# zwpku/colvars-finder

Measured on AMD Instinct MI355X. Metric: MD frames/sec through EigenFunctionTask train step, higher is better.
Workload: dtype f32; 1 GPU; BASELINE config 3: alanine-dipeptide-shaped EigenFunctionTask, generator mode, k=3, 22 atoms, align+position features d_r=66, nets [66,20,20,20,1], diag_coeff, Adam; frames_per_gpu=100000, batch_per_gpu=20000, global_batch=20000, parallelism=dp1 (frames sharded; all-reduce of batch sums + flat gradient)

## Files before the change

colvars-finder_amd/csrc/cvf_common.hpp:

```cpp
#pragma once
#include <hip/hip_runtime.h>
#include <stdint.h>
#include "cvf.h"

#define CVF_WAVE 64

void cvf_set_error(const char* fmt, ...);
int cvf_check_launch(const char* what);

#define CVF_REQUIRE(cond, ...)      \
  do {                              \
    if (!(cond)) {                  \
      cvf_set_error(__VA_ARGS__);   \
      return -1;                    \
    }                               \
  } while (0)

static inline int64_t cvf_ntiles(int64_t B) { return (B + CVF_TILE - 1) / CVF_TILE; }
static inline int cvf_cu_count() {
  static const int n = [] {
    int dev = 0, v = 0;
    if (hipGetDevice(&dev) != hipSuccess || hipDeviceGetAttribute(&v, hipDeviceAttributeMultiprocessorCount, dev) != hipSuccess || v < 1) v = 256;
    return v;
  }();
// ... 76 lines not shown

#ifdef CVF_STAMPS
#ifndef CVF_STAMP_WPB
#define CVF_STAMP_WPB 2
#endif
static __device__ unsigned long long g_stamps[64 * 4096];
#define CVF_STAMP(i)                                                                              \
  do {                                                                                            \
    if ((threadIdx.x & 63) == 0 && blockIdx.y == 0 && blockIdx.z == 0 && blockIdx.x < 4096 && (threadIdx.x >> 6) < CVF_STAMP_WPB)   \
      g_stamps[(blockIdx.x * CVF_STAMP_WPB + (threadIdx.x >> 6)) % 4096 * 64 + (i)] = __builtin_amdgcn_s_memtime(); \
  } while (0)
#define CVF_STAMP_RT(i)                                                                           \
  do {                                                                                            \
    if ((threadIdx.x & 63) == 0 && blockIdx.y == 0 && blockIdx.z == 0 && blockIdx.x < 4096 && (threadIdx.x >> 6) < CVF_STAMP_WPB)   \
      g_stamps[(blockIdx.x * CVF_STAMP_WPB + (threadIdx.x >> 6)) % 4096 * 64 + (i)] = __builtin_amdgcn_s_memrealtime(); \
  } while (0)
#else
#define CVF_STAMP(i) do {} while (0)
#define CVF_STAMP_RT(i) do {} while (0)
#endif

__host__ __device__ __forceinline__ int x_tile_stride(int nc) { return (nc & 3) == 2 ? nc : (nc | 1); }

template <int kBatch = 18>
__device__ __forceinline__ void load_x_tile(const float* __restrict__ x, int64_t B, int nc, int64_t tile, float* lds,
                                            int tid, int nthreads = CVF_WAVE, int frames = CVF_TILE) {
  const int stride = x_tile_stride(nc);
  const int64_t f0 = tile * frames;
  const int total = frames * nc;
  if (f0 + frames <= B) {
    const float4* src = reinterpret_cast<const float4*>(x + f0 * nc);
    const int nvec = total >> 2;
    int e = tid * 4;
    int fr = e / nc;
    int j = e - fr * nc;
    const int step = 4 * nthreads;
    const int dfr = step / nc, dj = step - dfr * nc;
    if (stride == nc) {
      float4* dst = reinterpret_cast<float4*>(lds);
      for (int v0 = tid; v0 < nvec; v0 += nthreads * kBatch) {
        float4 val[kBatch];
#pragma unroll
        for (int i = 0; i < kBatch; ++i) {
          const int v = v0 + nthreads * i;
          val[i] = src[v < nvec ? v : nvec - 1];
        }
#pragma unroll
// ... 9 lines not shown
#pragma unroll
      for (int i = 0; i < kBatch; ++i) {
        const int v = v0 + nthreads * i;
        val[i] = src[v < nvec ? v : nvec - 1];
      }
#pragma unroll
      for (int i = 0; i < kBatch; ++i) {
        if (v0 + nthreads * i < nvec) {
          int f = fr, jj = j;
          lds[f * stride + jj] = val[i].x;
          if (++jj == nc) { jj = 0; ++f; }
          lds[f * stride + jj] = val[i].y;
          if (++jj == nc) { jj = 0; ++f; }
          lds[f * stride + jj] = val[i].z;
          if (++jj == nc) { jj = 0; ++f; }
          lds[f * stride + jj] = val[i].w;
        }
        fr += dfr;
        j += dj;
        if (j >= nc) { j -= nc; ++fr; }
      }
    }
  } else {
    for (int e = tid; e < total; e += nthreads) {
      int fr = e / nc;
      int j = e - fr * nc;
      int64_t src = f0 + fr;
      if (src > B - 1) src = B - 1;
      lds[fr * stride + j] = x[src * nc + j];
    }
  }
}

__device__ __forceinline__ void lds_barrier() { asm volatile("s_waitcnt lgkmcnt(0)\n\ts_barrier" ::: "memory"); }

typedef float f2 __attribute__((ext_vector_type(2)));
__device__ __forceinline__ f2 splat2(float v) { return f2{v, v}; }
__device__ __forceinline__ f2 fma2(f2 a, f2 b, f2 c) { return __builtin_elementwise_fma(a, b, c); }

struct V3 {
  float x, y, z;
};
__device__ __forceinline__ V3 v3(float x, float y, float z) { return V3{x, y, z}; }
__device__ __forceinline__ V3 operator+(V3 a, V3 b) { return V3{a.x + b.x, a.y + b.y, a.z + b.z}; }
__device__ __forceinline__ V3 operator-(V3 a, V3 b) { return V3{a.x - b.x, a.y - b.y, a.z - b.z}; }
__device__ __forceinline__ V3 operator*(float s, V3 a) { return V3{s * a.x, s * a.y, s * a.z}; }
__device__ __forceinline__ float dot(V3 a, V3 b) { return a.x * b.x + a.y * b.y + a.z * b.z; }
__device__ __forceinline__ V3 cross(V3 a, V3 b) {
  return V3{a.y * b.z - a.z * b.y, a.z * b.x - a.x * b.z, a.x * b.y - a.y * b.x};
}

__device__ __forceinline__ V3 row_times(V3 v, const float* R) {
// ... 12 lines not shown
```

colvars-finder_amd/csrc/ef16_back.hip:

```cpp
#include "ef16_common.hpp"

namespace {

struct Back16Args {
  int k;
  int64_t B;
  int64_t n_tiles;
  int64_t T;
  const float* w_lag;
};
struct Back16Nets {
  int D;
  int n_params;
  int base[CVF_MAX_NETS];
};
template <int H, int NH>
__host__ __device__ constexpr int net_w_off(int l, int hd) { return l == 0 ? 0 : hd + H + (l - 1) * (H * H + H); }
template <int H, int NH>
__host__ __device__ constexpr int net_b_off(int l, int hd) { return net_w_off<H, NH>(l, hd) + (l == 0 ? hd : l == NH ? H : H * H); }

template <int H, int NH, bool MULTI, bool GEN>
__global__ __launch_bounds__(256, 4) void ef16_back_kernel(Back16Args args, Back16Nets nets, const float* __restrict__ theta,
                                                            const float* __restrict__ packed, const float* __restrict__ w,
                                                            const float* __restrict__ feat, const float* __restrict__ y_tiled,
// ... 111 lines not shown
  };

  int64_t tile = blockIdx.x;
  do {
    if constexpr (MULTI) {
      asm volatile("" : "+s"(D), "+s"(k));
      derive();
      asm volatile("" : "+v"(lane));
      derive_lane();
    }
    CVF_STAMP(8);
    double crow[CVF_MAX_NETS];
#pragma unroll
    for (int j = 0; j < CVF_MAX_NETS; ++j) crow[j] = coef[k + net * k + (j < k ? j : k - 1)];
    double gS1n = coef[net], gEtn = coef[k + k * k + net];
    double gS1ln = GEN ? 0.0 : coef[2 * k + k * k + net], gS2ln = GEN ? 0.0 : coef[3 * k + k * k + net];
    __builtin_amdgcn_sched_barrier(0);
    const bool lagged = !GEN && tile >= args.T;
    const int64_t t0 = lagged ? tile - args.T : tile;
    const int64_t frame = t0 * CVF_TILE + fo;
    const bool valid = frame < args.B;
    const float wraw = w[valid ? frame : args.B - 1];
    float yb[CVF_MAX_NETS];
#pragma unroll
    for (int j = 0; j < CVF_MAX_NETS; ++j) yb[j] = y_tiled[(t0 * k + (j < k ? j : k - 1)) * CVF_TILE + fo];
    float ylag = 0.0f, wlraw = 0.0f;
    if constexpr (!GEN) {
      ylag = y_tiled[((args.T + t0) * k + net) * CVF_TILE + fo];
      wlraw = args.w_lag[valid ? frame : args.B - 1];
    }
    const URows sv = urows(saved + (tile * k + net) * (int64_t)(kHand<NH>() * NG * 256) + wave * 64, kHand<NH>() * NG * 256 - wave * 64, lane);
    Vec<H, 1> h[NH], e[NH > 1 ? NH - 1 : 1], t[NH];
#pragma unroll
    for (int l = 0; l < NH; ++l) {
#pragma unroll
      for (int rt = 0; rt < RT; ++rt) h[l].v[rt][0] = f32x4{0.0f, 0.0f, 0.0f, 0.0f};
#pragma unroll
      for (int g = 0; g < NG; ++g) h[l].v[g >> 2][0][g & 3] = sv.ld((l * NG + g) * 256);
    }
    if constexpr (GEN) {
#pragma unroll
      for (int l = 0; l + 1 < NH; ++l) {
#pragma unroll
        for (int rt = 0; rt < RT; ++rt) e[l].v[rt][0] = f32x4{0.0f, 0.0f, 0.0f, 0.0f};
#pragma unroll
        for (int g = 0; g < NG; ++g) e[l].v[g >> 2][0][g & 3] = sv.ld(((NH + l) * NG + g) * 256);
      }
#pragma unroll
// ... 147 lines not shown
          for (int pr = wave; pr < RTO * CTH; pr += WPB) {
            const int rt = pr / CTH, ct = pr - rt * CTH;
            emit_tile(l, H, rt, ct, outer2(SA1, SB1, SA2, SB2, rt, ct));
          }
        }
        if (l == NH - 1) emit_last();
        __syncthreads();
      } else {
        if (strip) {
#pragma unroll
          for (int c = 0; c < 4; ++c) {
            if (c < ncol) {
              const float xv = c == nfeat ? 1.0f : xs[c < 3 ? c : 2];
              const float qv = c == nfeat ? 0.0f : gamma * qs[c < 3 ? c : 2];
              const float pick = strip_rows<H>([&](int rt, int r) {
                if constexpr (GEN) return fmaf(zbar.v[rt][0][r], xv, dl.v[rt][0][r] * qv);
                else return zbar.v[rt][0][r] * xv;
              }, col);
              if (col < NG && rowf < H) SB1[(wave * H + rowf) * 4 + c] = pick;
            }
          }
        }
        __syncthreads();
        auto half0 = [&](f32x4 (&acc)[RTO], const float* SA, const float4 (&b)[4], int ct, int rt0, int rstep, bool ones) {
          const int i = 16 * ct + row16;
          const float pad = (ones && i == D) ? 1.0f : 0.0f;
#pragma unroll
          for (int rt = 0; rt < RTO; ++rt) {
            if (rt >= rt0 && (rt - rt0) % rstep == 0) {
              const float4* a1 = reinterpret_cast<const float4*>(SA + (16 * rt + row16) * kPitch + 4 * q);
              float4 av[4];
#pragma unroll
              for (int j = 0; j < 4; ++j) av[j] = a1[4 * j];
#pragma unroll
              for (int j = 0; j < 4; ++j) {
                acc[rt] = mfma4(av[j].x, i < D ? b[j].x : pad, acc[rt]);
                acc[rt] = mfma4(av[j].y, i < D ? b[j].y : pad, acc[rt]);
                acc[rt] = mfma4(av[j].z, i < D ? b[j].z : pad, acc[rt]);
                acc[rt] = mfma4(av[j].w, i < D ? b[j].w : pad, acc[rt]);
              }
            }
          }
        };
        const int extra = (CTM - WPB) * RTO;
        f32x4 acc[RTO];
#pragma unroll
        for (int rt = 0; rt < RTO; ++rt) acc[rt] = f32x4{0.0f, 0.0f, 0.0f, 0.0f};
        auto tail0 = [&](f32x4& tacc, const float* SA, const float4 (&b)[4], int ct, bool ones) {
          const int i = 16 * ct + row16;
          const float pad = (ones && i == D) ? 1.0f : 0.0f;
          const float4* a1 = reinterpret_cast<const float4*>(SA + (16 + (lane & 3)) * kPitch + 4 * q);
          float4 av[4];
#pragma unroll
          for (int j = 0; j < 4; ++j) av[j] = a1[4 * j];
#pragma unroll
          for (int j = 0; j < 4; ++j) {
            tacc = mfma1(av[j].x, i < D ? b[j].x : pad, tacc);
            tacc = mfma1(av[j].y, i < D ? b[j].y : pad, tacc);
            tacc = mfma1(av[j].z, i < D ? b[j].z : pad, tacc);
            tacc = mfma1(av[j].w, i < D ? b[j].w : pad, tacc);
          }
        };
        if (wave < CTM) {
          f32x4 tacc = {0.0f, 0.0f, 0.0f, 0.0f};
          half0(acc, SA1, bA, wave, 0, TAIL4 ? RTO : 1, true);
          if constexpr (TAIL4) tail0(tacc, SA1, bA, wave, true);
          if (wave < extra) request(bA, f_tile, WPB + wave / RTO);
          if constexpr (GEN) {
            half0(acc, SA2, bB, wave, 0, TAIL4 ? RTO : 1, false);
            if constexpr (TAIL4) tail0(tacc, SA2, bB, wave, false);
          }
#pragma unroll
          for (int rt = 0; rt < (TAIL4 ? 1 : RTO); ++rt) emit_tile(0, D, rt, wave, acc[rt]);
          if constexpr (TAIL4) {
            const float v = rows_sum_scatter(tacc);
            int o = 16 + q;
            asm volatile("" : "+v"(o));
            const int i = 16 * wave + row16;
            const bool isw = o < H && i < D, isb = o < H && i == D;
            emit_entry(isw || isb, isw ? o * D + i : HD + (o < H ? o : 0), v);
          }
        }
        for (int pr = wave; pr < extra; pr += WPB) {
          const int ct = WPB + pr / RTO, rt = pr % RTO;
          if (pr != wave || wave >= CTM) request(bA, f_tile, ct);
          if constexpr (GEN) request(bB, q_tile, ct);
#pragma unroll
          for (int r_ = 0; r_ < RTO; ++r_) acc[r_] = f32x4{0.0f, 0.0f, 0.0f, 0.0f};
          half0(acc, SA1, bA, ct, rt, RTO, true);
          if constexpr (GEN) half0(acc, SA2, bB, ct, rt, RTO, false);
#pragma unroll
          for (int r_ = 0; r_ < RTO; ++r_)
            if (r_ == rt) emit_tile(0, D, r_, ct, acc[r_]);
        }
        emit_strip();
        if (NH == 1) emit_last();
        __syncthreads();
      }
    }
    tile += gridDim.x;
  } while (MULTI && tile < args.n_tiles);
  CVF_STAMP(17);
  if (MULTI) {
    __syncthreads();
    for (int i = tid; i < gspan; i += NT) out[i] = GI[i];
  }
  if (step != nullptr && blockIdx.x == 0 && blockIdx.y == 0 && tid == 0) *step += 1;
  CVF_STAMP(18);
}

}

extern "C" int64_t cvf_ef16_backward_slab_rows(int64_t n_tiles) { return n_tiles < 1024 ? n_tiles : 1024; }
// ... 74 lines not shown
```

colvars-finder_amd/csrc/ef16_front_kernel.hpp:

```cpp
#pragma once
#include "ef16_common.hpp"
#include "cvf_p2p.hpp"

namespace {
constexpr int kRowsUnit = kU * kAuxP;
static_assert(kRowsUnit % 4 == 0, "a unit's alignment rows are staged as 16-byte pieces");

template <bool kTransfer>
__device__ __forceinline__ void ef16_align_unit(const float* my, const float* refL, const int nal, const int lane, float* auxL,
                                                float* rsL) {
  const int f = lane >> 2, p = lane & 3;
  double acc[15];
#pragma unroll
  for (int i = 0; i < 15; ++i) acc[i] = 0.0;
#pragma unroll 2
  for (int b = p; b < nal; b += 4) {
    const double x0 = (double)my[3 * b], x1 = (double)my[3 * b + 1], x2 = (double)my[3 * b + 2];
    const double r0 = (double)refL[3 * b], r1 = (double)refL[3 * b + 1], r2 = (double)refL[3 * b + 2];
    acc[0] += x0; acc[1] += x1; acc[2] += x2;
    acc[3] = fma(x0, r0, acc[3]); acc[4] = fma(x0, r1, acc[4]); acc[5] = fma(x0, r2, acc[5]);
    acc[6] = fma(x1, r0, acc[6]); acc[7] = fma(x1, r1, acc[7]); acc[8] = fma(x1, r2, acc[8]);
    acc[9] = fma(x2, r0, acc[9]); acc[10] = fma(x2, r1, acc[10]); acc[11] = fma(x2, r2, acc[11]);
    acc[12] += r0; acc[13] += r1; acc[14] += r2;
  }
// ... 5 lines not shown
#pragma unroll
  for (int i = 0; i < 3; ++i)
#pragma unroll
    for (int j = 0; j < 3; ++j) Hm[i][j] = fma(-cd[i], acc[12 + j], acc[3 + 3 * i + j]);
  KabschOut ko;
  if constexpr (kTransfer) {
    kabsch_from_H<false>(Hm, ko);
#pragma unroll
    for (int i = 0; i < 6; ++i) ko.Kinv[i] = 0.0f;
  } else {
    kabsch_from_H<true>(Hm, ko);
  }
  const Centre c = centre_of(cd);
  const float av[kAuxP] = {ko.R[0], ko.R[1], ko.R[2], ko.R[3], ko.R[4], ko.R[5], ko.R[6], ko.R[7], ko.R[8], c.hi[0], c.hi[1], c.hi[2],
                           ko.Kinv[0], ko.Kinv[1], ko.Kinv[2], ko.Kinv[3], ko.Kinv[4], ko.Kinv[5], c.lo[0], c.lo[1], c.lo[2]};
#pragma unroll
  for (int i = 0; i < kAuxP; ++i)
    if ((i & 3) == p) auxL[f * kAuxP + i] = av[i];
  if (lane < 3) rsL[lane] = (float)(lane == 0 ? acc[12] : lane == 1 ? acc[13] : acc[14]);
}

__device__ __forceinline__ V3 ef16_feature(const float* my, const int at, const Centre& c, const float* R) {
  return row_times(centred(my, at, c), R);
}

template <int H, int NH, int NIT, bool ALLAL, bool ROWS = false>
__global__ __launch_bounds__(1024, 4) void ef16_front_kernel(cvf_mlp_desc mlp, const float* __restrict__ theta,
                                                             const float* __restrict__ packed, cvf_pp_desc pp,
                                                             const float* __restrict__ x, int64_t B,
                                                             const float* __restrict__ a, const float* __restrict__ w,
                                                             float* __restrict__ feat_tiled, float* __restrict__ y_tiled,
                                                             float* __restrict__ saved, float* __restrict__ q_tiled,
                                                             float* __restrict__ e_tiled, double* __restrict__ partial, int launch,
                                                             const float* __restrict__ x_lag, int64_t units_x,
                                                             const float* __restrict__ w_lag, const float* __restrict__ rows) {
  static_assert(!ROWS || NIT > 0, "alignment rows: generator instances only");
  constexpr int RT = Hid<H>::RT, NG = Hid<H>::NG, SMAX = 18, CTMAX = 5;
  constexpr bool kTransfer = NIT == 0;
  extern __shared__ __attribute__((aligned(16))) float lds_all[];
  const int upb = launch & 0xff;
  const int k = mlp.n_nets, D = mlp.dims[0];
  const int wave_b = __builtin_amdgcn_readfirstlane((int)threadIdx.x >> 6);
  const int usub = upb > 1 ? wave_b / k : 0;
  const int wave = wave_b - usub * k;
  const int tid = (int)threadIdx.x - usub * (64 * k), lane_in = tid & 63;
  const int nthreads = upb > 1 ? 64 * k : (int)blockDim.x, nw = nthreads >> 6;
// ... 74 lines not shown
    const int64_t frame = unit * kU + (tid < kU ? tid : kU - 1);
    const float wv_ld = *(w != nullptr ? w + (frame < B ? frame : B - 1) : rows);
    const float wv = (w != nullptr && frame < B) ? wv_ld : 0.0f;
    {
      const float* ft = feat_tiled + tile * (int64_t)D * CVF_TILE + kU * sub + col;
#pragma unroll
      for (int s = 0; s < SMAX; ++s) {
        const int kf = 4 * (s < S ? s : S - 1) + q;
        bf0[s] = ft[(kf < D ? kf : D - 1) * CVF_TILE];
      }
    }
    request_a0();
    float4* adst = reinterpret_cast<float4*>(auxL);
    if (tid < n4r) adst[tid] = row_a;
    if (tid + nthreads < n4r) adst[tid + nthreads] = row_b;
    if (tid < 3) rsL[tid] = rs_in;
    if (iso) {
    } else if (plain) {
      float4* dst = reinterpret_cast<float4*>(xt);
      if (tid < n4) dst[tid] = cx0;
      if (tid + nthreads < n4) dst[tid + nthreads] = cx1;
      for (int v = tid + 2 * nthreads; v < n4; v += nthreads) dst[v] = xsrc[v];
    } else {
      load_x_tile<6>(x, B, nc, unit, xt, tid, nthreads, kU);
    }
    if (tid < nt) refL[tid] = tv;
    for (int j = tid + nthreads; j < nt; j += nthreads) refL[j] = j < 3 * nal ? pp.ref_c[j] : (a != nullptr ? a[j - 3 * nal] : 0.0f);
    if (tid < kU) wL[tid] = wv;
    request_bias0();
  } else {
  if (stride == nc && (unit + 1) * kU <= B && (reinterpret_cast<uintptr_t>(x) & 15) == 0) {
    const float4* src = reinterpret_cast<const float4*>(x + unit * (int64_t)(kU * nc));
    float4* dst = reinterpret_cast<float4*>(xt);
    const int n4 = (kU * nc) >> 2;
    for (int v = tid; v < n4; v += nthreads) dst[v] = src[v];
  } else {
    load_x_tile<6>(x, B, nc, unit, xt, tid, nthreads, kU);
  }
  for (int j = tid; j < 3 * nal + nc; j += nthreads) refL[j] = j < 3 * nal ? pp.ref_c[j] : (a != nullptr ? a[j - 3 * nal] : 0.0f);
  if (tid < kU) {
    const int64_t frame = unit * kU + tid;
    wL[tid] = (w != nullptr && frame < B) ? w[frame] : 0.0f;
  }
  if (wave != 0) request_layer0();
  __syncthreads();
  }
  const float* my = xt + f * stride;
// ... 6 lines not shown
    }
    lds_barrier();
  }
  CVF_STAMP(22);

  if constexpr (!ROWS) {
    float R[9];
    const float* ar = auxL + f * kAuxP;
#pragma unroll
    for (int i = 0; i < 9; ++i) R[i] = ar[i];
    Centre c;
#pragma unroll
    for (int i = 0; i < 3; ++i) {
      c.hi[i] = ar[9 + i];
      c.lo[i] = ar[18 + i];
    }
    for (int at = p + 4 * wave; at < N; at += 4 * nw) {
      const V3 al = ef16_feature(my, at, c, R);
      float* fi = featI + f * kImgP + 3 * at;
      fi[0] = al.x;
      fi[1] = al.y;
      fi[2] = al.z;
    }
    lds_barrier();
  }
  CVF_STAMP(23);

  Vec<H, 1> h[NH];
  auto set_bias = [&](Vec<H, 1>& X, const float (&b)[RT][4]) {
#pragma unroll
    for (int rt = 0; rt < RT; ++rt)
#pragma unroll
      for (int r = 0; r < 4; ++r) X.v[rt][0][r] = b[rt][r];
  };
  set_bias(h[0], bias[0]);
  {
    float bf[SMAX];
    float* fr = featI + col * kImgP;
    static_assert(4 * (SMAX - 1) + 3 < kImgP, "the ROWS twins' feature copy stays inside a frame's row of the image");
    unsigned own = 0u;
    if constexpr (ROWS) {
      if (iso) {
        const int P = nw >= 8 ? 8 : nw >= 4 ? 4 : nw >= 2 ? 2 : 1;
        own = (P == 8 ? 0x10101u : P == 4 ? 0x11111u : P == 2 ? 0x15555u : 0x3ffffu) << (wave & (P - 1));
      }
    }
#pragma unroll
    for (int s = 0; s < SMAX; ++s) {
      const int kf = 4 * (s < S ? s : S - 1) + q;
      if constexpr (ROWS) bf[s] = bf0[s];
      else bf[s] = fr[kf < D ? kf : D - 1];
    }
    HFrag<H> hf[NH > 1 ? NH - 1 : 1];
#pragma unroll
    for (int l = 1; l < NH; ++l) {
      load_hfrag_u<H>(hf[l - 1], pk, L.fh(l));
      load_hid_const_u<H>(urows(theta + mlp.b_off[net][l], H, q), bias[l]);
    }
#pragma unroll
    for (int s = 0; s < SMAX; ++s) {
      if (s < S) {
#pragma unroll
        for (int rt = 0; rt < RT; ++rt) h[0].v[rt][0] = mfma4(a0[s][rt], bf[s], h[0].v[rt][0]);
        if constexpr (ROWS) {
          if ((own >> s) & 1u) fr[q + 4 * s] = bf[s];
        }
      }
    }
    CVF_STAMP(24);
    tanh_inplace<H, 1>(h[0]);
#pragma unroll
    for (int l = 1; l < NH; ++l) {
      set_bias(h[l], bias[l]);
      hidden_mul<H, 1>(h[l], hf[l - 1], h[l - 1]);
      tanh_inplace<H, 1>(h[l]);
    }
  }
  float wl[RT][4];
  load_hid_const_u<H>(urows(theta + mlp.w_off[net][NH], H, q), wl);
  const float bL = theta[mlp.b_off[net][NH]];
  HFrag<H> tf[NH > 1 ? NH - 1 : 1];
#pragma unroll
  for (int l = 1; l < NH; ++l) load_hfrag_u<H>(tf[l - 1], pk, L.th(l));

  const URows sv = urows(saved + (tile * k + net) * (int64_t)(kHand<NH>() * NG * 256) + sub * 64, kHand<NH>() * NG * 256 - sub * 64, lane);
  {
    float part = 0.0f;
#pragma unroll
    for (int rt = 0; rt < RT; ++rt)
#pragma unroll
      for (int r = 0; r < 4; ++r) part = fmaf(wl[rt][r], h[NH - 1].v[rt][0][r], part);
    const float yv = sum_over_q(part) + bL;
    yL[net * kU + col] = yv;
    y_tiled[(tile * k + net) * CVF_TILE + kU * sub + col] = yv;
  }
  CVF_STAMP(25);
  if constexpr (kTransfer) {
#pragma unroll
    for (int l = 0; l < NH; ++l)
#pragma unroll
      for (int g = 0; g < NG; ++g) sv.st((l * NG + g) * 256, h[l].v[g >> 2][0][g & 3]);
    float* ft = feat_tiled + tile * (int64_t)D * CVF_TILE + kU * sub + f;
    const float* fi = featI + f * kImgP;
#pragma unroll 1
    for (int j = p + 4 * wave; j < D; j += 4 * nw) ft[j * CVF_TILE] = fi[j];
    return;
  } else {

  {
    float t0[CTMAX][NG];
#pragma unroll
    for (int rt = 0; rt < CTMAX; ++rt)
#pragma unroll
      for (int s = 0; s < NG; ++s) t0[rt][s] = pk.ld(L.t0() + ((rt < CT ? rt : CT - 1) * NG + s) * 64);
    Vec<H, 1> d;
#pragma unroll
    for (int rt = 0; rt < RT; ++rt)
// ... 19 lines not shown
      }
    }
#pragma unroll
    for (int l = 0; l < NH; ++l)
#pragma unroll
      for (int g = 0; g < NG; ++g) sv.st((l * NG + g) * 256, h[l].v[g >> 2][0][g & 3]);
#pragma unroll
    for (int l = 1; l < NH; ++l)
#pragma unroll
      for (int g = 0; g < NG; ++g) sv.st(((NH + l - 1) * NG + g) * 256, ev[l - 1].v[g >> 2][0][g & 3]);
  }
  if constexpr (ROWS) lds_barrier();
  CVF_STAMP(26);
  asm volatile("s_waitcnt lgkmcnt(0)" ::: "memory");

  float f0b[SMAX][RT];
  {
    const float* ar = auxL + f * kAuxP;
    float* Ul = gI + f * kImgP;
    V3 gv[NIT];
    if (iso) {
    const float* Fl = featI + f * kImgP;
    V3 gsum = v3(0.0f, 0.0f, 0.0f), tau = v3(0.0f, 0.0f, 0.0f);
#pragma unroll
    for (int it = 0; it < NIT; ++it) {
      int at = p + 4 * it;
      asm volatile("" : "+v"(at));
      const bool last = it == NIT - 1;
      const int ac = (last && at >= N) ? N - 1 : at;
      const float lv = (last && at >= N) ? 0.0f : 1.0f;
      gv[it] = v3(Ul[3 * ac], Ul[3 * ac + 1], Ul[3 * ac + 2]);
      const V3 fb = v3(Fl[3 * ac], Fl[3 * ac + 1], Fl[3 * ac + 2]);
      const V3 gm = last ? lv * gv[it] : gv[it];
      gsum = gsum + gm;
      tau.x = fmaf(gm.y, fb.z, fmaf(-gm.z, fb.y, tau.x));
      tau.y = fmaf(gm.z, fb.x, fmaf(-gm.x, fb.z, tau.y));
      tau.z = fmaf(gm.x, fb.y, fmaf(-gm.y, fb.x, tau.z));
    }
    CVF_STAMP(27);
    gsum = v3(quad_sumf16(gsum.x), quad_sumf16(gsum.y), quad_sumf16(gsum.z));
    tau = v3(quad_sumf16(tau.x), quad_sumf16(tau.y), quad_sumf16(tau.z));
    float Kinv[6];
#pragma unroll
    for (int i = 0; i < 6; ++i) Kinv[i] = ar[12 + i];
    const V3 s = sym_times(Kinv, tau);
    const float inv_nal = 1.0f / (float)nal;
    const V3 gbar = inv_nal * gsum;
    float E = 0.0f;
    V3 usum = v3(0.0f, 0.0f, 0.0f), tau2 = v3(0.0f, 0.0f, 0.0f);
#pragma unroll
    for (int it = 0; it < NIT; ++it) {
      int at = p + 4 * it;
      asm volatile("" : "+v"(at));
      const bool last = it == NIT - 1;
      const int ac = (last && at >= N) ? N - 1 : at;
      const float lv = (last && at >= N) ? 0.0f : 1.0f;
      const float ma = ALLAL ? 1.0f : (ac < nal ? 1.0f : 0.0f);
      const int ar_ = ALLAL ? ac : (ac < nal ? ac : 0);
      V3 rf = v3(refL[3 * ar_], refL[3 * ar_ + 1], refL[3 * ar_ + 2]);
      if (!ALLAL) rf = ma * rf;
      const V3 sh = ALLAL ? gbar : ma * gbar;
      V3 G;
      G.x = fmaf(s.y, rf.z, fmaf(-s.z, rf.y, gv[it].x - sh.x));
      G.y = fmaf(s.z, rf.x, fmaf(-s.x, rf.z, gv[it].y - sh.y));
      G.z = fmaf(s.x, rf.y, fmaf(-s.y, rf.x, gv[it].z - sh.z));
      const V3 u = aL[3 * ac] * G;
      gv[it] = u;
      const bool masked = last || !ALLAL;
      const V3 ue = last ? lv * u : u;
      E = fmaf(ue.x, G.x, fmaf(ue.y, G.y, fmaf(ue.z, G.z, E)));
      const V3 um = masked ? (ma * lv) * u : u;
      usum = usum + um;
      tau2.x = fmaf(rf.y, um.z, fmaf(-rf.z, um.y, tau2.x));
      tau2.y = fmaf(rf.z, um.x, fmaf(-rf.x, um.z, tau2.y));
      tau2.z = fmaf(rf.x, um.y, fmaf(-rf.y, um.x, tau2.z));
    }
    CVF_STAMP(28);
    E = quad_sumf16(E);
    usum = v3(quad_sumf16(usum.x), quad_sumf16(usum.y), quad_sumf16(usum.z));
    tau2 = v3(quad_sumf16(tau2.x), quad_sumf16(tau2.y), quad_sumf16(tau2.z));
    const V3 rsum = v3(rsL[0], rsL[1], rsL[2]);
    eL[net * kU + f] = E;
    e_tiled[(tile * k + net) * CVF_TILE + kU * sub + f] = E;
    const V3 ubar = inv_nal * usum;
    tau2.x = fmaf(-rsum.y, ubar.z, fmaf(rsum.z, ubar.y, tau2.x));
    tau2.y = fmaf(-rsum.z, ubar.x, fmaf(rsum.x, ubar.z, tau2.y));
    tau2.z = fmaf(-rsum.x, ubar.y, fmaf(rsum.y, ubar.x, tau2.z));
    const V3 om = sym_times(Kinv, tau2);
    CVF_STAMP(31);
#pragma unroll
    for (int it = 0; it < NIT; ++it) {
      int at = p + 4 * it;
      asm volatile("" : "+v"(at));
      const int ac = (it == NIT - 1 && at >= N) ? N - 1 : at;
      const V3 fb = v3(Fl[3 * ac], Fl[3 * ac + 1], Fl[3 * ac + 2]);
      V3 qv;
      qv.x = fmaf(fb.y, om.z, fmaf(-fb.z, om.y, gv[it].x - ubar.x));
      qv.y = fmaf(fb.z, om.x, fmaf(-fb.x, om.z, gv[it].y - ubar.y));
      qv.z = fmaf(fb.x, om.y, fmaf(-fb.y, om.x, gv[it].z - ubar.z));
      gv[it] = qv;
      Ul[3 * ac] = qv.x;
      Ul[3 * ac + 1] = qv.y;
      Ul[3 * ac + 2] = qv.z;
    }
    } else {
    float R[9];
#pragma unroll
    for (int i = 0; i < 9; ++i) R[i] = ar[i];
    const Centre c = centre_of(ar[9], ar[10], ar[11]);
    V3 gsum = v3(0.0f, 0.0f, 0.0f);
    Outer3 Mo = {{{0.0f, 0.0f}, {0.0f, 0.0f}, {0.0f, 0.0f}}, {0.0f, 0.0f, 0.0f}};
#pragma unroll
    for (int it = 0; it < NIT; ++it) {
      int at = p + 4 * it;
      asm volatile("" : "+v"(at));
      const bool last = it == NIT - 1;
      const int ac = (last && at >= N) ? N - 1 : at;
      const float lv = (last && at >= N) ? 0.0f : 1.0f;
      gv[it] = v3(Ul[3 * ac], Ul[3 * ac + 1], Ul[3 * ac + 2]);
      const V3 gm = last ? lv * gv[it] : gv[it];
      gsum = gsum + gm;
      outer_acc(Mo, centred(my, ac, c), gm);
    }
    CVF_STAMP(27);
    gsum = v3(quad_sumf16(gsum.x), quad_sumf16(gsum.y), quad_sumf16(gsum.z));
    const V3 sump = mat_times(R, gsum);
    float M[9];
    outer_to_array(Mo, M);
#pragma unroll
    for (int i = 0; i < 9; ++i) M[i] = quad_sumf16(M[i]);
    float T[9], Z[9];
#pragma unroll
    for (int i = 0; i < 3; ++i)
#pragma unroll
      for (int j = 0; j < 3; ++j) T[3 * i + j] = R[i] * M[j] + R[3 + i] * M[3 + j] + R[6 + i] * M[6 + j];
    float Kinv[6];
#pragma unroll
    for (int i = 0; i < 6; ++i) Kinv[i] = ar[12 + i];
    const V3 s = sym_times(Kinv, v3(T[7] - T[5], T[2] - T[6], T[3] - T[1]));
#pragma unroll
    for (int i = 0; i < 3; ++i) {
      Z[3 * i + 0] = R[3 * i + 1] * s.z - R[3 * i + 2] * s.y;
      Z[3 * i + 1] = -R[3 * i + 0] * s.z + R[3 * i + 2] * s.x;
      Z[3 * i + 2] = R[3 * i + 0] * s.y - R[3 * i + 1] * s.x;
    }
    const float inv_nal = 1.0f / (float)nal;
    const V3 shift = inv_nal * sump;
    const MatCols Rc = mat_cols(R), Zc = mat_cols(Z);
    f2 E2 = {0.0f, 0.0f};
    float Ez = 0.0f;
    f2 usum_xy = {0.0f, 0.0f};
    float usum_z = 0.0f;
    Outer3 dHo = {{{0.0f, 0.0f}, {0.0f, 0.0f}, {0.0f, 0.0f}}, {0.0f, 0.0f, 0.0f}};
#pragma unroll
    for (int it = 0; it < NIT; ++it) {
      int at = p + 4 * it;
      asm volatile("" : "+v"(at));
      const bool last = it == NIT - 1;
      const int ac = (last && at >= N) ? N - 1 : at;
      const float lv = (last && at >= N) ? 0.0f : 1.0f;
      const float ma = ALLAL ? 1.0f : (ac < nal ? 1.0f : 0.0f);
      const int ar_ = ALLAL ? ac : (ac < nal ? ac : 0);
      V3 rf = v3(refL[3 * ar_], refL[3 * ar_ + 1], refL[3 * ar_ + 2]);
      if (!ALLAL) rf = ma * rf;
      f2 Gxy = ALLAL ? f2{-shift.x, -shift.y} : f2{-ma * shift.x, -ma * shift.y};
      float Gz = ALLAL ? -shift.z : -ma * shift.z;
      mat_times_acc(Rc, gv[it], Gxy, Gz);
      mat_times_acc(Zc, rf, Gxy, Gz);
      const f2 uxy = f2{aL[3 * ac], aL[3 * ac + 1]} * Gxy;
      const float uz = aL[3 * ac + 2] * Gz;
      gv[it] = v3(uxy.x, uxy.y, uz);
      const bool masked = last || !ALLAL;
      const float m = ma * lv;
      const f2 uxm = masked ? m * uxy : uxy;
      const float uzm = masked ? m * uz : uz;
      E2 = fma2(last ? lv * uxy : uxy, Gxy, E2);
      Ez = fmaf(last ? lv * uz : uz, Gz, Ez);
      usum_xy += uxm; usum_z += uzm;
      outer_acc(dHo, v3(uxm.x, uxm.y, uzm), rf);
    }
    CVF_STAMP(28);
    const float E = quad_sumf16((E2.x + E2.y) + Ez);
    const V3 usum = v3(quad_sumf16(usum_xy.x), quad_sumf16(usum_xy.y), quad_sumf16(usum_z));
    const V3 rsum = v3(rsL[0], rsL[1], rsL[2]);
    float dH[9];
    outer_to_array(dHo, dH);
#pragma unroll
    for (int i = 0; i < 9; ++i) dH[i] = quad_sumf16(dH[i]);
    eL[net * kU + f] = E;
    e_tiled[(tile * k + net) * CVF_TILE + kU * sub + f] = E;
    const V3 ubar = inv_nal * usum;
    dH[0] -= ubar.x * rsum.x; dH[1] -= ubar.x * rsum.y; dH[2] -= ubar.x * rsum.z;
    dH[3] -= ubar.y * rsum.x; dH[4] -= ubar.y * rsum.y; dH[5] -= ubar.y * rsum.z;
    dH[6] -= ubar.z * rsum.x; dH[7] -= ubar.z * rsum.y; dH[8] -= ubar.z * rsum.z;
#pragma unroll
    for (int i = 0; i < 3; ++i)
#pragma unroll
      for (int j = 0; j < 3; ++j) T[3 * i + j] = R[i] * dH[j] + R[3 + i] * dH[3 + j] + R[6 + i] * dH[6 + j];
    asm volatile("" ::: "memory");
#pragma unroll
    for (int i = 0; i < 6; ++i) Kinv[i] = ar[12 + i];
    const V3 om = sym_times(Kinv, v3(T[7] - T[5], T[2] - T[6], T[3] - T[1]));
    float dR[9];
#pragma unroll
    for (int i = 0; i < 3; ++i) {
      dR[3 * i + 0] = R[3 * i + 1] * om.z - R[3 * i + 2] * om.y;
      dR[3 * i + 1] = -R[3 * i + 0] * om.z + R[3 * i + 2] * om.x;
      dR[3 * i + 2] = R[3 * i + 0] * om.y - R[3 * i + 1] * om.x;
    }
    CVF_STAMP(31);
    const MatRows Rr = mat_rows(R), dRr = mat_rows(dR);
#pragma unroll
    for (int it = 0; it < NIT; ++it) {
      int at = p + 4 * it;
      asm volatile("" : "+v"(at));
      const int ac = (it == NIT - 1 && at >= N) ? N - 1 : at;
      f2 qxy = {0.0f, 0.0f};
      float qz = 0.0f;
      row_times_acc(Rr, gv[it] - ubar, qxy, qz);
      row_times_acc(dRr, centred(my, ac, c), qxy, qz);
      gv[it] = v3(qxy.x, qxy.y, qz);
      Ul[3 * ac] = qxy.x;
      Ul[3 * ac + 1] = qxy.y;
      Ul[3 * ac + 2] = qz;
    }
    }
    CVF_STAMP(32);
    asm volatile("" ::: "memory");
#pragma unroll
    for (int s_ = 0; s_ < SMAX; ++s_) {
      const int se = s_ < S ? s_ : S - 1;
#pragma unroll
      for (int rt = 0; rt < RT; ++rt) f0b[s_][rt] = pk.ld(L.f0() + (se * RT + rt) * 64);
    }
    {
      asm volatile("s_waitcnt lgkmcnt(0)" ::: "memory");
      Vec<H, 1> sv0;
      init_bias<H, 1>(sv0, nullptr, q);
      const float* qr = gI + col * kImgP;
#pragma unroll
      for (int s = 0; s < SMAX; ++s) {
        if (s < S) {
          const int kf = 4 * s + q;
          const float b = qr[kf < D ? kf : D - 1];
#pragma unroll
          for (int rt = 0; rt < RT; ++rt) sv0.v[rt][0] = mfma4(f0b[s][rt], b, sv0.v[rt][0]);
        }
      }
#pragma unroll
      for (int g = 0; g < NG; ++g) sv.st(((2 * NH - 1) * NG + g) * 256, sv0.v[g >> 2][0][g & 3]);
    }
    CVF_STAMP(33);
    float* qt = q_tiled + (tile * k + net) * (int64_t)D * CVF_TILE + kU * sub + f;
#pragma unroll
    for (int it = 0; it < NIT; ++it) {
      int at = p + 4 * it;
      asm volatile("" : "+v"(at));
      const int ac = (it == NIT - 1 && at >= N) ? N - 1 : at;
      qt[(3 * ac) * CVF_TILE] = gv[it].x;
      qt[(3 * ac + 1) * CVF_TILE] = gv[it].y;
      qt[(3 * ac + 2) * CVF_TILE] = gv[it].z;
    }
  }
  CVF_STAMP(34);
  if constexpr (!ROWS) {
    float* ft = feat_tiled + tile * (int64_t)D * CVF_TILE + kU * sub + f;
    const float* fi = featI + f * kImgP;
#pragma unroll 1
    for (int j = p + 4 * wave; j < D; j += 4 * nw) ft[j * CVF_TILE] = fi[j];
  }
  CVF_STAMP(29);
  if (partial == nullptr) return;
  lds_barrier();

  if (wave == 0) {
    typedef double f64x4 __attribute__((ext_vector_type(4)));
    const int np = CVF_NPAIR(k);
    const int i = lane & 15, kq = lane >> 4;
    f64x4 d1 = {0.0, 0.0, 0.0, 0.0}, d2 = {0.0, 0.0, 0.0, 0.0};
    const float* yrow = yL + (i >= 1 && i <= k ? i - 1 : 0) * kU;
    const float* erow = eL + (i < k ? i : 0) * kU;
#pragma unroll
    for (int s_ = 0; s_ < 4; ++s_) {
      const int fr = 4 * s_ + kq;
      const double wb = (double)wL[fr];
      const double yv = (double)yrow[fr];
      const double a1 = i == 0 ? 1.0 : (i <= k ? yv : 0.0);
      const double b = i == 0 ? wb : (i <= k ? wb * yv : 0.0);
      const double a2 = i < k ? (double)erow[fr] : 0.0;
      d1 = __builtin_amdgcn_mfma_f64_16x16x4f64(a1, b, d1, 0, 0, 0);
      d2 = __builtin_amdgcn_mfma_f64_16x16x4f64(a2, b, d2, 0, 0, 0);
    }
    const int cj = lane & 15;
    const int64_t G = units_x;
#pragma unroll
    for (int r = 0; r < 4; ++r) {
      const int ri = (lane >> 4) + 4 * r;
      int t = -1;
      if (ri == 0 && cj <= k) t = cj;
      else if (ri >= 1 && ri <= cj && cj <= k) {
        const int a_ = ri - 1, b_ = cj - 1;
        t = 1 + k + a_ * k - (a_ * (a_ - 1)) / 2 + (b_ - a_);
      }
      if (t >= 0) partial[t * G + unit] = d1[r];
      if (cj == 0 && ri < k) partial[(1 + k + np + ri) * G + unit] = d2[r];
    }
  }
  CVF_STAMP(30);
  }
  };
  run_pass(0);
  if constexpr (kTransfer) {
    if (!paired) return;
    run_pass(1);
    if (partial == nullptr) return;
    const int lane = lane_in;
    const int64_t unit = ub;
    lds_barrier();
    if (wave == 0) {
      typedef double f64x4 __attribute__((ext_vector_type(4)));
      const int np = CVF_NPAIR(k);
      const int i = lane & 15, kq = lane >> 4;
      const float* y0 = lds + Lo.y;
      const float* y1 = y0 + k * kU;
      const float* w0 = lds + Lo.w;
      const float* w1 = lds + Lo.g;
      f64x4 d1 = {0.0, 0.0, 0.0, 0.0}, d2 = {0.0, 0.0, 0.0, 0.0}, d3 = {0.0, 0.0, 0.0, 0.0};
      const int yi = (i >= 1 && i <= k ? i - 1 : 0) * kU, ti = (i < k ? i : 0) * kU;
// ... 109 lines not shown
```

Baseline: 352.9 million frames/s.

## Streamline index math, padding, and stores across front and back kernels

Several micro-optimizations land together. Atom indices are precomputed through an AtomSlot helper so only the last iteration gets clamped. The feature image is zero-padded so the clamping on feature loads can be dropped. Pad selection in the backward MFMA loop is skipped when a tile is full, stores of y/e/q and of partial sums go through buffer-resource stores that discard out-of-range writes, and the ragged x-load batch size is reduced. The aim is fewer VALU selects and address computations, at the cost of relying on out-of-bounds buffer stores being dropped and on the added zero padding being correct.

After: 357.3 million frames/s, median of 6. 1.01x the previous value.

```diff
diff --git a/colvars-finder_amd/csrc/cvf_common.hpp b/colvars-finder_amd/csrc/cvf_common.hpp
--- a/colvars-finder_amd/csrc/cvf_common.hpp
+++ b/colvars-finder_amd/csrc/cvf_common.hpp
@@ -122,7 +122,7 @@
 
 __host__ __device__ __forceinline__ int x_tile_stride(int nc) { return (nc & 3) == 2 ? nc : (nc | 1); }
 
-template <int kBatch = 18>
+template <int kBatch = 18, bool kPlainRagged = false>
 __device__ __forceinline__ void load_x_tile(const float* __restrict__ x, int64_t B, int nc, int64_t tile, float* lds,
                                             int tid, int nthreads = CVF_WAVE, int frames = CVF_TILE) {
   const int stride = x_tile_stride(nc);
@@ -178,12 +178,18 @@
       }
     }
   } else {
-    for (int e = tid; e < total; e += nthreads) {
+    auto one = [&](const int e) {
       int fr = e / nc;
       int j = e - fr * nc;
       int64_t src = f0 + fr;
       if (src > B - 1) src = B - 1;
       lds[fr * stride + j] = x[src * nc + j];
+    };
+    if constexpr (kPlainRagged) {
+#pragma unroll 1
+      for (int e = tid; e < total; e += nthreads) one(e);
+    } else {
+      for (int e = tid; e < total; e += nthreads) one(e);
     }
   }
 }
diff --git a/colvars-finder_amd/csrc/ef16_back.hip b/colvars-finder_amd/csrc/ef16_back.hip
--- a/colvars-finder_amd/csrc/ef16_back.hip
+++ b/colvars-finder_amd/csrc/ef16_back.hip
@@ -157,8 +157,14 @@
     const bool valid = frame < args.B;
     const float wraw = w[valid ? frame : args.B - 1];
     float yb[CVF_MAX_NETS];
-#pragma unroll
-    for (int j = 0; j < CVF_MAX_NETS; ++j) yb[j] = y_tiled[(t0 * k + (j < k ? j : k - 1)) * CVF_TILE + fo];
+    if constexpr (MULTI) {
+#pragma unroll
+      for (int j = 0; j < CVF_MAX_NETS; ++j) yb[j] = y_tiled[(t0 * k + (j < k ? j : k - 1)) * CVF_TILE + fo];
+    } else {
+      const URows yrows = urows(y_tiled + t0 * k * CVF_TILE, k * CVF_TILE, fo);
+#pragma unroll
+      for (int j = 0; j < CVF_MAX_NETS; ++j) yb[j] = yrows.ld(j * CVF_TILE);
+    }
     float ylag = 0.0f, wlraw = 0.0f;
     if constexpr (!GEN) {
       ylag = y_tiled[((args.T + t0) * k + net) * CVF_TILE + fo];
@@ -352,9 +358,14 @@
           }
         }
         __syncthreads();
-        auto half0 = [&](f32x4 (&acc)[RTO], const float* SA, const float4 (&b)[4], int ct, int rt0, int rstep, bool ones) {
+        auto pad_rows = [&](float4 (&b)[4], int ct, bool ones) {
+          if (!MULTI && 16 * ct + 16 <= D) return;
           const int i = 16 * ct + row16;
           const float pad = (ones && i == D) ? 1.0f : 0.0f;
+#pragma unroll
+          for (int j = 0; j < 4; ++j) b[j] = float4{i < D ? b[j].x : pad, i < D ? b[j].y : pad, i < D ? b[j].z : pad, i < D ? b[j].w : pad};
+        };
+        auto half0 = [&](f32x4 (&acc)[RTO], const float* SA, const float4 (&b)[4], int rt0, int rstep) {
 #pragma unroll
           for (int rt = 0; rt < RTO; ++rt) {
             if (rt >= rt0 && (rt - rt0) % rstep == 0) {
@@ -364,10 +375,10 @@
               for (int j = 0; j < 4; ++j) av[j] = a1[4 * j];
 #pragma unroll
               for (int j = 0; j < 4; ++j) {
-                acc[rt] = mfma4(av[j].x, i < D ? b[j].x : pad, acc[rt]);
-                acc[rt] = mfma4(av[j].y, i < D ? b[j].y : pad, acc[rt]);
-                acc[rt] = mfma4(av[j].z, i < D ? b[j].z : pad, acc[rt]);
-                acc[rt] = mfma4(av[j].w, i < D ? b[j].w : pad, acc[rt]);
+                acc[rt] = mfma4(av[j].x, b[j].x, acc[rt]);
+                acc[rt] = mfma4(av[j].y, b[j].y, acc[rt]);
+                acc[rt] = mfma4(av[j].z, b[j].z, acc[rt]);
+                acc[rt] = mfma4(av[j].w, b[j].w, acc[rt]);
               }
             }
           }
@@ -376,29 +387,29 @@
         f32x4 acc[RTO];
 #pragma unroll
         for (int rt = 0; rt < RTO; ++rt) acc[rt] = f32x4{0.0f, 0.0f, 0.0f, 0.0f};
-        auto tail0 = [&](f32x4& tacc, const float* SA, const float4 (&b)[4], int ct, bool ones) {
-          const int i = 16 * ct + row16;
-          const float pad = (ones && i == D) ? 1.0f : 0.0f;
+        auto tail0 = [&](f32x4& tacc, const float* SA, const float4 (&b)[4]) {
           const float4* a1 = reinterpret_cast<const float4*>(SA + (16 + (lane & 3)) * kPitch + 4 * q);
           float4 av[4];
 #pragma unroll
           for (int j = 0; j < 4; ++j) av[j] = a1[4 * j];
 #pragma unroll
           for (int j = 0; j < 4; ++j) {
-            tacc = mfma1(av[j].x, i < D ? b[j].x : pad, tacc);
-            tacc = mfma1(av[j].y, i < D ? b[j].y : pad, tacc);
-            tacc = mfma1(av[j].z, i < D ? b[j].z : pad, tacc);
-            tacc = mfma1(av[j].w, i < D ? b[j].w : pad, tacc);
+            tacc = mfma1(av[j].x, b[j].x, tacc);
+            tacc = mfma1(av[j].y, b[j].y, tacc);
+            tacc = mfma1(av[j].z, b[j].z, tacc);
+            tacc = mfma1(av[j].w, b[j].w, tacc);
           }
         };
         if (wave < CTM) {
           f32x4 tacc = {0.0f, 0.0f, 0.0f, 0.0f};
-          half0(acc, SA1, bA, wave, 0, TAIL4 ? RTO : 1, true);
-          if constexpr (TAIL4) tail0(tacc, SA1, bA, wave, true);
+          pad_rows(bA, wave, true);
+          half0(acc, SA1, bA, 0, TAIL4 ? RTO : 1);
+          if constexpr (TAIL4) tail0(tacc, SA1, bA);
           if (wave < extra) request(bA, f_tile, WPB + wave / RTO);
           if constexpr (GEN) {
-            half0(acc, SA2, bB, wave, 0, TAIL4 ? RTO : 1, false);
-            if constexpr (TAIL4) tail0(tacc, SA2, bB, wave, false);
+            pad_rows(bB, wave, false);
+            half0(acc, SA2, bB, 0, TAIL4 ? RTO : 1);
+            if constexpr (TAIL4) tail0(tacc, SA2, bB);
           }
 #pragma unroll
           for (int rt = 0; rt < (TAIL4 ? 1 : RTO); ++rt) emit_tile(0, D, rt, wave, acc[rt]);
@@ -417,8 +428,12 @@
           if constexpr (GEN) request(bB, q_tile, ct);
 #pragma unroll
           for (int r_ = 0; r_ < RTO; ++r_) acc[r_] = f32x4{0.0f, 0.0f, 0.0f, 0.0f};
-          half0(acc, SA1, bA, ct, rt, RTO, true);
-          if constexpr (GEN) half0(acc, SA2, bB, ct, rt, RTO, false);
+          pad_rows(bA, ct, true);
+          half0(acc, SA1, bA, rt, RTO);
+          if constexpr (GEN) {
+            pad_rows(bB, ct, false);
+            half0(acc, SA2, bB, rt, RTO);
+          }
 #pragma unroll
           for (int r_ = 0; r_ < RTO; ++r_)
             if (r_ == rt) emit_tile(0, D, r_, ct, acc[r_]);
diff --git a/colvars-finder_amd/csrc/ef16_front_kernel.hpp b/colvars-finder_amd/csrc/ef16_front_kernel.hpp
--- a/colvars-finder_amd/csrc/ef16_front_kernel.hpp
+++ b/colvars-finder_amd/csrc/ef16_front_kernel.hpp
@@ -51,6 +51,19 @@
 
 __device__ __forceinline__ V3 ef16_feature(const float* my, const int at, const Centre& c, const float* R) {
   return row_times(centred(my, at, c), R);
+}
+
+struct AtomSlot {
+  int ac, i3;
+  float lv;
+};
+template <int NIT>
+__device__ __forceinline__ AtomSlot atom_slot(const int pb, const int it, const int N) {
+  asm volatile("");
+  const int at = pb + 4 * it;
+  if (it < NIT - 1) return AtomSlot{at, 3 * pb + 12 * it, 1.0f};
+  const int ac = at >= N ? N - 1 : at;
+  return AtomSlot{ac, 3 * ac, at >= N ? 0.0f : 1.0f};
 }
 
 template <int H, int NH, int NIT, bool ALLAL, bool ROWS = false>
@@ -171,7 +184,7 @@
       if (tid + nthreads < n4) dst[tid + nthreads] = cx1;
       for (int v = tid + 2 * nthreads; v < n4; v += nthreads) dst[v] = xsrc[v];
     } else {
-      load_x_tile<6>(x, B, nc, unit, xt, tid, nthreads, kU);
+      load_x_tile<3, true>(x, B, nc, unit, xt, tid, nthreads, kU);
     }
     if (tid < nt) refL[tid] = tv;
     for (int j = tid + nthreads; j < nt; j += nthreads) refL[j] = j < 3 * nal ? pp.ref_c[j] : (a != nullptr ? a[j - 3 * nal] : 0.0f);
@@ -224,6 +237,7 @@
       fi[1] = al.y;
       fi[2] = al.z;
     }
+    if (wave == 0 && D + p < 4 * S) featI[f * kImgP + D + p] = 0.0f;
     lds_barrier();
   }
   CVF_STAMP(23);
@@ -249,9 +263,8 @@
     }
 #pragma unroll
     for (int s = 0; s < SMAX; ++s) {
-      const int kf = 4 * (s < S ? s : S - 1) + q;
       if constexpr (ROWS) bf[s] = bf0[s];
-      else bf[s] = fr[kf < D ? kf : D - 1];
+      else bf[s] = fr[q + 4 * s];
     }
     HFrag<H> hf[NH > 1 ? NH - 1 : 1];
 #pragma unroll
@@ -294,7 +307,7 @@
       for (int r = 0; r < 4; ++r) part = fmaf(wl[rt][r], h[NH - 1].v[rt][0][r], part);
     const float yv = sum_over_q(part) + bL;
     yL[net * kU + col] = yv;
-    y_tiled[(tile * k + net) * CVF_TILE + kU * sub + col] = yv;
+    urows(y_tiled + (tile * k + net) * CVF_TILE + kU * sub, kU, col).st(0, yv);
   }
   CVF_STAMP(25);
   if constexpr (kTransfer) {
@@ -360,15 +373,16 @@
     if (iso) {
     const float* Fl = featI + f * kImgP;
     V3 gsum = v3(0.0f, 0.0f, 0.0f), tau = v3(0.0f, 0.0f, 0.0f);
+    int pb = p;
+    asm volatile("" : "+v"(pb));
 #pragma unroll
     for (int it = 0; it < NIT; ++it) {
-      int at = p + 4 * it;
-      asm volatile("" : "+v"(at));
+      const AtomSlot sl = atom_slot<NIT>(pb, it, N);
       const bool last = it == NIT - 1;
-      const int ac = (last && at >= N) ? N - 1 : at;
-      const float lv = (last && at >= N) ? 0.0f : 1.0f;
-      gv[it] = v3(Ul[3 * ac], Ul[3 * ac + 1], Ul[3 * ac + 2]);
-      const V3 fb = v3(Fl[3 * ac], Fl[3 * ac + 1], Fl[3 * ac + 2]);
+      const int i3 = sl.i3;
+      const float lv = sl.lv;
+      gv[it] = v3(Ul[i3], Ul[i3 + 1], Ul[i3 + 2]);
+      const V3 fb = v3(Fl[i3], Fl[i3 + 1], Fl[i3 + 2]);
       const V3 gm = last ? lv * gv[it] : gv[it];
       gsum = gsum + gm;
       tau.x = fmaf(gm.y, fb.z, fmaf(-gm.z, fb.y, tau.x));
@@ -386,23 +400,24 @@
     const V3 gbar = inv_nal * gsum;
     float E = 0.0f;
     V3 usum = v3(0.0f, 0.0f, 0.0f), tau2 = v3(0.0f, 0.0f, 0.0f);
+    pb = p;
+    asm volatile("" : "+v"(pb));
 #pragma unroll
     for (int it = 0; it < NIT; ++it) {
-      int at = p + 4 * it;
-      asm volatile("" : "+v"(at));
+      const AtomSlot sl = atom_slot<NIT>(pb, it, N);
       const bool last = it == NIT - 1;
-      const int ac = (last && at >= N) ? N - 1 : at;
-      const float lv = (last && at >= N) ? 0.0f : 1.0f;
+      const int ac = sl.ac;
+      const float lv = sl.lv;
       const float ma = ALLAL ? 1.0f : (ac < nal ? 1.0f : 0.0f);
-      const int ar_ = ALLAL ? ac : (ac < nal ? ac : 0);
-      V3 rf = v3(refL[3 * ar_], refL[3 * ar_ + 1], refL[3 * ar_ + 2]);
+      const int r3 = ALLAL ? sl.i3 : (ac < nal ? sl.i3 : 0);
+      V3 rf = v3(refL[r3], refL[r3 + 1], refL[r3 + 2]);
       if (!ALLAL) rf = ma * rf;
       const V3 sh = ALLAL ? gbar : ma * gbar;
       V3 G;
       G.x = fmaf(s.y, rf.z, fmaf(-s.z, rf.y, gv[it].x - sh.x));
       G.y = fmaf(s.z, rf.x, fmaf(-s.x, rf.z, gv[it].y - sh.y));
       G.z = fmaf(s.x, rf.y, fmaf(-s.y, rf.x, gv[it].z - sh.z));
-      const V3 u = aL[3 * ac] * G;
+      const V3 u = aL[sl.i3] * G;
       gv[it] = u;
       const bool masked = last || !ALLAL;
       const V3 ue = last ? lv * u : u;
@@ -419,27 +434,27 @@
     tau2 = v3(quad_sumf16(tau2.x), quad_sumf16(tau2.y), quad_sumf16(tau2.z));
     const V3 rsum = v3(rsL[0], rsL[1], rsL[2]);
     eL[net * kU + f] = E;
-    e_tiled[(tile * k + net) * CVF_TILE + kU * sub + f] = E;
+    urows(e_tiled + (tile * k + net) * CVF_TILE + kU * sub, kU, f).st(0, E);
     const V3 ubar = inv_nal * usum;
     tau2.x = fmaf(-rsum.y, ubar.z, fmaf(rsum.z, ubar.y, tau2.x));
     tau2.y = fmaf(-rsum.z, ubar.x, fmaf(rsum.x, ubar.z, tau2.y));
     tau2.z = fmaf(-rsum.x, ubar.y, fmaf(rsum.y, ubar.x, tau2.z));
     const V3 om = sym_times(Kinv, tau2);
     CVF_STAMP(31);
+    pb = p;
+    asm volatile("" : "+v"(pb));
 #pragma unroll
     for (int it = 0; it < NIT; ++it) {
-      int at = p + 4 * it;
-      asm volatile("" : "+v"(at));
-      const int ac = (it == NIT - 1 && at >= N) ? N - 1 : at;
-      const V3 fb = v3(Fl[3 * ac], Fl[3 * ac + 1], Fl[3 * ac + 2]);
+      const int i3 = atom_slot<NIT>(pb, it, N).i3;
+      const V3 fb = v3(Fl[i3], Fl[i3 + 1], Fl[i3 + 2]);
       V3 qv;
       qv.x = fmaf(fb.y, om.z, fmaf(-fb.z, om.y, gv[it].x - ubar.x));
       qv.y = fmaf(fb.z, om.x, fmaf(-fb.x, om.z, gv[it].y - ubar.y));
       qv.z = fmaf(fb.x, om.y, fmaf(-fb.y, om.x, gv[it].z - ubar.z));
       gv[it] = qv;
-      Ul[3 * ac] = qv.x;
-      Ul[3 * ac + 1] = qv.y;
-      Ul[3 * ac + 2] = qv.z;
+      Ul[i3] = qv.x;
+      Ul[i3 + 1] = qv.y;
+      Ul[i3 + 2] = qv.z;
     }
     } else {
     float R[9];
@@ -448,17 +463,18 @@
     const Centre c = centre_of(ar[9], ar[10], ar[11]);
     V3 gsum = v3(0.0f, 0.0f, 0.0f);
     Outer3 Mo = {{{0.0f, 0.0f}, {0.0f, 0.0f}, {0.0f, 0.0f}}, {0.0f, 0.0f, 0.0f}};
+    int pb = p;
+    asm volatile("" : "+v"(pb));
 #pragma unroll
     for (int it = 0; it < NIT; ++it) {
-      int at = p + 4 * it;
-      asm volatile("" : "+v"(at));
+      const AtomSlot sl = atom_slot<NIT>(pb, it, N);
       const bool last = it == NIT - 1;
-      const int ac = (last && at >= N) ? N - 1 : at;
-      const float lv = (last && at >= N) ? 0.0f : 1.0f;
-      gv[it] = v3(Ul[3 * ac], Ul[3 * ac + 1], Ul[3 * ac + 2]);
+      const int i3 = sl.i3;
+      const float lv = sl.lv;
+      gv[it] = v3(Ul[i3], Ul[i3 + 1], Ul[i3 + 2]);
       const V3 gm = last ? lv * gv[it] : gv[it];
       gsum = gsum + gm;
-      outer_acc(Mo, centred(my, ac, c), gm);
+      outer_acc(Mo, centred(my + i3, 0, c), gm);
     }
     CVF_STAMP(27);
     gsum = v3(quad_sumf16(gsum.x), quad_sumf16(gsum.y), quad_sumf16(gsum.z));
@@ -490,23 +506,25 @@
     f2 usum_xy = {0.0f, 0.0f};
     float usum_z = 0.0f;
     Outer3 dHo = {{{0.0f, 0.0f}, {0.0f, 0.0f}, {0.0f, 0.0f}}, {0.0f, 0.0f, 0.0f}};
+    pb = p;
+    asm volatile("" : "+v"(pb));
 #pragma unroll
     for (int it = 0; it < NIT; ++it) {
-      int at = p + 4 * it;
-      asm volatile("" : "+v"(at));
+      const AtomSlot sl = atom_slot<NIT>(pb, it, N);
       const bool last = it == NIT - 1;
-      const int ac = (last && at >= N) ? N - 1 : at;
-      const float lv = (last && at >= N) ? 0.0f : 1.0f;
+      const int ac = sl.ac, i3 = sl.i3;
+      const float lv = sl.lv;
       const float ma = ALLAL ? 1.0f : (ac < nal ? 1.0f : 0.0f);
-      const int ar_ = ALLAL ? ac : (ac < nal ? ac : 0);
-      V3 rf = v3(refL[3 * ar_], refL[3 * ar_ + 1], refL[3 * ar_ + 2]);
+      const int r3 = ALLAL ? i3 : (ac < nal ? i3 : 0);
+      V3 rf = v3(refL[r3], refL[r3 + 1], refL[r3 + 2]);
       if (!ALLAL) rf = ma * rf;
       f2 Gxy = ALLAL ? f2{-shift.x, -shift.y} : f2{-ma * shift.x, -ma * shift.y};
       float Gz = ALLAL ? -shift.z : -ma * shift.z;
       mat_times_acc(Rc, gv[it], Gxy, Gz);
       mat_times_acc(Zc, rf, Gxy, Gz);
-      const f2 uxy = f2{aL[3 * ac], aL[3 * ac + 1]} * Gxy;
-      const float uz = aL[3 * ac + 2] * Gz;
+      asm volatile("");
+      const f2 uxy = f2{aL[i3], aL[i3 + 1]} * Gxy;
+      const float uz = aL[i3 + 2] * Gz;
       gv[it] = v3(uxy.x, uxy.y, uz);
       const bool masked = last || !ALLAL;
       const float m = ma * lv;
@@ -526,7 +544,7 @@
 #pragma unroll
     for (int i = 0; i < 9; ++i) dH[i] = quad_sumf16(dH[i]);
     eL[net * kU + f] = E;
-    e_tiled[(tile * k + net) * CVF_TILE + kU * sub + f] = E;
+    urows(e_tiled + (tile * k + net) * CVF_TILE + kU * sub, kU, f).st(0, E);
     const V3 ubar = inv_nal * usum;
     dH[0] -= ubar.x * rsum.x; dH[1] -= ubar.x * rsum.y; dH[2] -= ubar.x * rsum.z;
     dH[3] -= ubar.y * rsum.x; dH[4] -= ubar.y * rsum.y; dH[5] -= ubar.y * rsum.z;
@@ -548,26 +566,28 @@
     }
     CVF_STAMP(31);
     const MatRows Rr = mat_rows(R), dRr = mat_rows(dR);
+    pb = p;
+    asm volatile("" : "+v"(pb));
 #pragma unroll
     for (int it = 0; it < NIT; ++it) {
-      int at = p + 4 * it;
-      asm volatile("" : "+v"(at));
-      const int ac = (it == NIT - 1 && at >= N) ? N - 1 : at;
+      const int i3 = atom_slot<NIT>(pb, it, N).i3;
       f2 qxy = {0.0f, 0.0f};
       float qz = 0.0f;
       row_times_acc(Rr, gv[it] - ubar, qxy, qz);
-      row_times_acc(dRr, centred(my, ac, c), qxy, qz);
+      row_times_acc(dRr, centred(my + i3, 0, c), qxy, qz);
       gv[it] = v3(qxy.x, qxy.y, qz);
-      Ul[3 * ac] = qxy.x;
-      Ul[3 * ac + 1] = qxy.y;
-      Ul[3 * ac + 2] = qz;
+      Ul[i3] = qxy.x;
+      Ul[i3 + 1] = qxy.y;
+      Ul[i3 + 2] = qz;
     }
     }
     CVF_STAMP(32);
     asm volatile("" ::: "memory");
+    int Sq = S;
+    asm volatile("" : "+s"(Sq));
 #pragma unroll
     for (int s_ = 0; s_ < SMAX; ++s_) {
-      const int se = s_ < S ? s_ : S - 1;
+      const int se = s_ < Sq ? s_ : Sq - 1;
 #pragma unroll
       for (int rt = 0; rt < RT; ++rt) f0b[s_][rt] = pk.ld(L.f0() + (se * RT + rt) * 64);
     }
@@ -575,12 +595,11 @@
       asm volatile("s_waitcnt lgkmcnt(0)" ::: "memory");
       Vec<H, 1> sv0;
       init_bias<H, 1>(sv0, nullptr, q);
-      const float* qr = gI + col * kImgP;
+      const float* qr = gI + col * kImgP + q;
 #pragma unroll
       for (int s = 0; s < SMAX; ++s) {
-        if (s < S) {
-          const int kf = 4 * s + q;
-          const float b = qr[kf < D ? kf : D - 1];
+        if (s < Sq) {
+          const float b = qr[4 * s];
 #pragma unroll
           for (int rt = 0; rt < RT; ++rt) sv0.v[rt][0] = mfma4(f0b[s][rt], b, sv0.v[rt][0]);
         }
@@ -589,15 +608,19 @@
       for (int g = 0; g < NG; ++g) sv.st(((2 * NH - 1) * NG + g) * 256, sv0.v[g >> 2][0][g & 3]);
     }
     CVF_STAMP(33);
-    float* qt = q_tiled + (tile * k + net) * (int64_t)D * CVF_TILE + kU * sub + f;
+    const int q_floats = D * CVF_TILE - kU * sub;
+    const __amdgpu_buffer_rsrc_t qres =
+        __builtin_amdgcn_make_buffer_rsrc(q_tiled + (tile * k + net) * (int64_t)D * CVF_TILE + kU * sub, 0, q_floats * 4, 0x00020000);
+    int pb = p;
+    asm volatile("" : "+v"(pb));
 #pragma unroll
     for (int it = 0; it < NIT; ++it) {
-      int at = p + 4 * it;
-      asm volatile("" : "+v"(at));
-      const int ac = (it == NIT - 1 && at >= N) ? N - 1 : at;
-      qt[(3 * ac) * CVF_TILE] = gv[it].x;
-      qt[(3 * ac + 1) * CVF_TILE] = gv[it].y;
-      qt[(3 * ac + 2) * CVF_TILE] = gv[it].z;
+      const bool last = it == NIT - 1;
+      const URows qt{qres, ((last ? atom_slot<NIT>(pb, it, N).i3 : 3 * pb) * CVF_TILE + f) * 4};
+      const int row = last ? 0 : 12 * it;
+      qt.st(row * CVF_TILE, gv[it].x);
+      qt.st((row + 1) * CVF_TILE, gv[it].y);
+      qt.st((row + 2) * CVF_TILE, gv[it].z);
     }
   }
   CVF_STAMP(34);
@@ -609,6 +632,18 @@
   }
   CVF_STAMP(29);
   if (partial == nullptr) return;
+  constexpr int kDeadRow = 0x7fff0000;
+  int o1[4], o2[4];
+  if (wave == 0) {
+    const int cj = lane & 15, G = (int)units_x, u = (int)unit;
+#pragma unroll
+    for (int r = 0; r < 4; ++r) {
+      const int ri = (lane >> 4) + 4 * r, a_ = ri - 1;
+      const int t = ri == 0 ? cj : 1 + k + __mul24(a_, k) - (__mul24(a_, a_ - 1) >> 1) + (cj - ri);
+      o1[r] = (ri <= cj && cj <= k) ? (__mul24(t, G) + u) * 8 : kDeadRow;
+      o2[r] = (cj == 0 && ri < k) ? (__mul24(1 + k + CVF_NPAIR(k) + ri, G) + u) * 8 : kDeadRow;
+    }
+  }
   lds_barrier();
 
   if (wave == 0) {
@@ -629,19 +664,13 @@
       d1 = __builtin_amdgcn_mfma_f64_16x16x4f64(a1, b, d1, 0, 0, 0);
       d2 = __builtin_amdgcn_mfma_f64_16x16x4f64(a2, b, d2, 0, 0, 0);
     }
-    const int cj = lane & 15;
-    const int64_t G = units_x;
+    typedef unsigned u32x2 __attribute__((ext_vector_type(2)));
+    const __amdgpu_buffer_rsrc_t pres = __builtin_amdgcn_make_buffer_rsrc(partial, 0, __mul24(1 + 2 * k + np, (int)units_x) * 8, 0x00020000);
 #pragma unroll
     for (int r = 0; r < 4; ++r) {
-      const int ri = (lane >> 4) + 4 * r;
-      int t = -1;
-      if (ri == 0 && cj <= k) t = cj;
-      else if (ri >= 1 && ri <= cj && cj <= k) {
-        const int a_ = ri - 1, b_ = cj - 1;
-        t = 1 + k + a_ * k - (a_ * (a_ - 1)) / 2 + (b_ - a_);
-      }
-      if (t >= 0) partial[t * G + unit] = d1[r];
-      if (cj == 0 && ri < k) partial[(1 + k + np + ri) * G + unit] = d2[r];
+      const double v1 = d1[r], v2 = d2[r];
+      __builtin_amdgcn_raw_buffer_store_b64(__builtin_bit_cast(u32x2, v1), pres, o1[r], 0, 0);
+      __builtin_amdgcn_raw_buffer_store_b64(__builtin_bit_cast(u32x2, v2), pres, o2[r], 0, 0);
     }
   }
   CVF_STAMP(30);
```
